# qiyunzhu/woltka

Hardware: AMD Instinct MI355X
Metric: alignment records/sec classified (higher is better)
Workload: dtype u8; 1 GPU; synthetic SAM text of 50M reads x <=16 hits (10.50 GB) resident in HBM, 2M-node taxonomy, ranks phylum,genus,species: device tokenizer per 64 MB block + one weighted histogram per sample (the kernels of `woltka classify`, host link left out); records_per_gpu=250034804, reads_per_gpu=50000000

## Files before the change

woltka_amd/csrc/wk_dtok_fused.hpp:

```cpp
#pragma once
#include "wk_dtok.hpp"
#include "wk_dtok_neighbour.hpp"
#include "wk_dtok_planes.hpp"
#include "wk_dtok_rounds.hpp"

namespace wk {

constexpr uint32_t kFzThreads = 512;
constexpr uint32_t kFzWaves = kFzThreads / kWave;
constexpr uint32_t kFzTile = 16384;
constexpr uint32_t kFzBack = 1024;
constexpr uint32_t kFzFwd = 3072;
constexpr uint32_t kFzWin = kFzTile + kFzBack + kFzFwd;
constexpr uint32_t kFzChunks = kFzWin / 16 + 1;
constexpr uint32_t kFzRounds = kFrMaxRounds;
static_assert(kFrChunks * 16u == kFzWin && kFrTailChunk + 1u == kFzChunks && kFrWaves == kFzWaves && kFrWave == kWave,
              "the dealing covers the window");
constexpr uint32_t kFzLines = 1024;
constexpr uint32_t kFzStreams = 4;
constexpr uint32_t kFzCap = 1024;
static_assert(kFzCap >= kFzLines, "a window's records fit an empty buffer");
static_assert(kFzWin + 32 < 65536, "window offsets fit 16 bits");
constexpr uint32_t kFzCarry = 256;
static_assert(kFzCarry + kFzLines <= kFpMaxLines && kFzThreads % kWave == 0, "a window's owned lines fit the planes, a wave's lines one word");

constexpr uint32_t kDtokSpill = 64;

struct FusedArgs {
    const unsigned char* text;
    uint32_t n;
    uint32_t open_end;
    uint32_t span;
    const struct DictSlot8* dict8;
    const uint4* names16;
    uint32_t dict_mask;
    const unsigned char* arena;
    uint2* unknown;
    uint32_t unknown_cap;
    DtokState* state;
    DtokState* host_state;
    const unsigned long long* backup_prev;
    unsigned long long* backup_next;
    uint32_t* host_seq;
    uint32_t seq;
    StreamSet streams;
    const int32_t* submap;
    uint32_t n_submap;
    uint32_t ablate;
};

static_assert(sizeof(DtokState) % 8 == 0, "the packed totals are aligned");
__device__ __forceinline__ unsigned long long* fz_totals(DtokState* state) { return reinterpret_cast<unsigned long long*>(state + 1); }

__global__ void dtok_fused_begin_kernel(unsigned long long* __restrict__ backup, const unsigned long long* __restrict__ cursor, DtokState* state) {
    if (threadIdx.x < (uint32_t)kMaxStreams) backup[threadIdx.x] = cursor[threadIdx.x];
    if (threadIdx.x == 0) {
        *state = DtokState{0u, 0u, 0ull, 0ull, 0ull, 0u, 0u};
        *fz_totals(state) = 0ull;
    }
}

template <int kCtrl, int kRowMask>
__device__ __forceinline__ uint32_t fz_dpp_add(uint32_t v) {
    return v + (uint32_t)__builtin_amdgcn_update_dpp(0, (int)v, kCtrl, kRowMask, 0xF, false);
}
__device__ __forceinline__ uint32_t fz_wave_scan(uint32_t v) {
    static_assert(kWave == 64, "four rows of sixteen lanes");
    v = fz_dpp_add<0x111, 0xF>(v);
    v = fz_dpp_add<0x112, 0xF>(v);
    v = fz_dpp_add<0x114, 0xF>(v);
    v = fz_dpp_add<0x118, 0xF>(v);
    v = fz_dpp_add<0x142, 0xA>(v);
    v = fz_dpp_add<0x143, 0xC>(v);
    return v;
}
__device__ __forceinline__ uint32_t fz_last_lane(uint32_t v) { return (uint32_t)__builtin_amdgcn_readlane((int)v, kWave - 1); }
__device__ __forceinline__ uint32_t fz_wave_sum(uint32_t v) { return fz_last_lane(fz_wave_scan(v)); }
__device__ __forceinline__ unsigned long long fz_first_lane64(unsigned long long v) {
    return ((unsigned long long)(uint32_t)__builtin_amdgcn_readfirstlane((int)(uint32_t)(v >> 32)) << 32) |
           (uint32_t)__builtin_amdgcn_readfirstlane((int)(uint32_t)v);
}

__device__ __forceinline__ uint4 fz_load_stream(const unsigned char* p) {
    typedef uint32_t u32x4 __attribute__((ext_vector_type(4)));
    const u32x4 v = __builtin_nontemporal_load(reinterpret_cast<const u32x4*>(p));
    return make_uint4(v.x, v.y, v.z, v.w);
}
__device__ __forceinline__ unsigned long long fz_load64(const unsigned char* p) {
    unsigned long long w;
    __builtin_memcpy(&w, p, 8);
    return w;
}
__device__ __forceinline__ uint32_t fz_load32(const unsigned char* p) {
    uint32_t w;
    __builtin_memcpy(&w, p, 4);
    return w;
}
__device__ __forceinline__ unsigned long long fz_eq_bytes(unsigned long long w, unsigned char c) {
    const unsigned long long x = w ^ (0x0101010101010101ull * c);
    return ~(((x & 0x7F7F7F7F7F7F7F7Full) + 0x7F7F7F7F7F7F7F7Full) | x | 0x7F7F7F7F7F7F7F7Full);
}
__device__ __forceinline__ uint32_t fz_marks32(uint32_t w, uint32_t c4) {
    const uint32_t x = w ^ c4;
    return ~(((x & 0x7F7F7F7Fu) + 0x7F7F7F7Fu) | x | 0x7F7F7F7Fu);
}
__device__ __forceinline__ unsigned long long fz_low_bytes(unsigned long long w, uint32_t k) {
    return k >= 8u ? w : (w & ((1ull << (8u * k)) - 1ull));
}

__device__ __forceinline__ unsigned long long fz_hash(const unsigned char* p, uint32_t n) {
    unsigned long long h = 0xcbf29ce484222325ull ^ ((unsigned long long)n * 0x9E3779B97F4A7C15ull);
    while (n >= 8u) {
        h = (h ^ fz_load64(p)) * 0x100000001b3ull;
        h ^= h >> 29;
        p += 8;
        n -= 8u;
    }
    const unsigned long long v = n ? fz_low_bytes(fz_load64(p), n) : 0ull;
    h = (h ^ v) * 0x100000001b3ull;
    h ^= h >> 32;
    h *= 0x9E3779B97F4A7C15ull;
    return h ^ (h >> 29);
}

__device__ __forceinline__ bool fz_same(const unsigned char* x, const unsigned char* y, uint32_t n) {
    while (n >= 8u) {
        if (fz_load64(x) != fz_load64(y)) return false;
        x += 8;
        y += 8;
        n -= 8u;
    }
    return n == 0u || fz_low_bytes(fz_load64(x) ^ fz_load64(y), n) == 0ull;
}

struct FzProbe {
    unsigned long long hv, n0, n1;
    uint32_t h;
    uint2 slot;
};
__device__ __forceinline__ FzProbe fz_probe_begin(const FusedArgs& a, const unsigned char* name, uint32_t rn) {
    FzProbe p;
    p.n0 = p.n1 = 0ull;
    if (rn <= 15u) {
        const unsigned long long lo = fz_low_bytes(fz_load64(name), rn), hi = rn > 8u ? fz_low_bytes(fz_load64(name + 8), rn - 8u) : 0ull;
        p.n0 = lo;
        p.n1 = hi | ((unsigned long long)rn << 56);
        unsigned long long h = 0xcbf29ce484222325ull ^ ((unsigned long long)rn * 0x9E3779B97F4A7C15ull), v = lo;
        if (rn >= 8u) {
            h = (h ^ lo) * 0x100000001b3ull;
            h ^= h >> 29;
            v = hi;
        }
        h = (h ^ v) * 0x100000001b3ull;
        h ^= h >> 32;
        h *= 0x9E3779B97F4A7C15ull;
        p.hv = h ^ (h >> 29);
    } else {
        p.hv = fz_hash(name, rn);
    }
    p.h = (uint32_t)p.hv & a.dict_mask;
    p.slot = reinterpret_cast<const uint2*>(a.dict8)[p.h];
    return p;
}
__device__ __forceinline__ int32_t fz_probe_end(const FusedArgs& a, FzProbe p, const unsigned char* name, uint32_t rn, uint32_t abs_off) {
    for (;;) {
        const int32_t id = (int32_t)p.slot.y;
        if (id < 0) break;
        if (p.slot.x == (uint32_t)(p.hv >> 32)) {
            const uint4 nm = a.names16[id];
            const unsigned long long s0 = ((unsigned long long)nm.y << 32) | nm.x, s1 = ((unsigned long long)nm.w << 32) | nm.z;
            if (rn <= 15u) {
                if (s0 == p.n0 && s1 == p.n1) return id;
            } else if ((nm.w >> 24) == 0xFFu) {
                const unsigned char* full = a.arena + nm.x;
                if (fz_load32(full) == rn && fz_same(name, full + 4, rn)) return id;
            }
        }
        p.h = (p.h + 1u) & a.dict_mask;
        p.slot = reinterpret_cast<const uint2*>(a.dict8)[p.h];
    }
    const uint32_t at = atomicAdd(&a.state->n_unknown, 1u);
    if (at < a.unknown_cap)
        a.unknown[at] = make_uint2(abs_off, rn);
    else
        atomicOr(&a.state->flags, kDtokUnknownFull);
    return kLineUnknown;
}

__device__ bool fz_starts_run_slow(const unsigned char* __restrict__ text, uint32_t at, const unsigned char* q, uint32_t qn) {
    uint32_t pos = at;
    while (pos > 0u) {
        const uint32_t e = pos - 1u;
        uint32_t s = e;
        while (s > 0u && text[s - 1u] != '\n') --s;
        uint32_t tab[3], nt = 0;
        for (uint32_t p = s; p < e && nt < 3u; ++p)
            if (text[p] == '\t') tab[nt++] = p;
        if (nt == 3u && !(tab[2] - tab[1] == 2u && text[tab[1] + 1u] == '*')) {
            if (tab[0] - s != qn) return true;
            for (uint32_t k = 0; k < qn; ++k)
                if (text[s + k] != q[k]) return true;
            return false;
        }
        pos = s;
    }
    return true;
}

constexpr uint32_t kFiSubj = (1u << 23) - 1u;
constexpr uint32_t kFiMateShift = 24;
constexpr uint32_t kFiMapped = 1u << 26;
constexpr uint32_t kFiStart = 1u << 27;
constexpr uint32_t kFiUndecided = 1u << 28;
constexpr uint32_t kFiExcl = 1u << 29;
constexpr uint32_t kFiDropped = 1u << 30;
constexpr uint32_t kFiRead = kFiMapped | (3u << kFiMateShift);
constexpr uint32_t kFiKey = kFiRead | kFiSubj;
constexpr uint32_t kFzPad = 8;
static_assert(kFwWave == kWave && kFwWaves == kFzWaves, "the line pass's dealing is this workgroup's");

__device__ __forceinline__ uint32_t fz_octet(uint32_t z_lo, uint32_t z_hi) { return (((z_lo >> 7) | (z_hi >> 3)) * 0x00204081u >> 21) & 255u; }

__device__ __forceinline__ uint32_t fz_newlines16(uint4 v) {
    return fz_octet(fz_marks32(v.x, 0x0A0A0A0Au), fz_marks32(v.y, 0x0A0A0A0Au)) | (fz_octet(fz_marks32(v.z, 0x0A0A0A0Au), fz_marks32(v.w, 0x0A0A0A0Au)) << 8);
}

__device__ __forceinline__ uint32_t fz_tabs32(const unsigned char* p, unsigned long long* q0 = nullptr, unsigned long long* q1 = nullptr) {
    unsigned long long w[4];
#pragma unroll
    for (uint32_t i = 0; i < 4; ++i) w[i] = fz_load64(p + 8u * i);
    uint32_t m = 0;
#pragma unroll
    for (uint32_t i = 0; i < 4; ++i)
        m |= fz_octet(fz_marks32((uint32_t)w[i], 0x09090909u), fz_marks32((uint32_t)(w[i] >> 32), 0x09090909u)) << (8u * i);
    if (q0) {
        *q0 = w[0];
        *q1 = w[1];
    }
    return m;
}

template <bool kMeasure>
__device__ __forceinline__ void dtok_fused_body(const FusedArgs& a) {
    __shared__ __attribute__((aligned(16))) unsigned char txt[kFzChunks * 16 + 32];
    __shared__ uint16_t ls[kFzLines + 2];
    __shared__ uint16_t f_qn[kFzLines];
    __shared__ __attribute__((aligned(16))) uint32_t info_[kFzPad + kFzCarry + kFzLines + kFzPad + 8];
    __shared__ uint32_t carry[kFzCarry];
    __shared__ unsigned long long planes[kFpPlanes][kFpWords];
    __shared__ uint32_t rbuf[kFzStreams][kFzCap];
    __shared__ unsigned long long fill_packed;
    static_assert(kFzStreams <= 4 && kFzCap + kFzThreads < 65536, "four 16-bit counts");
    __shared__ unsigned long long gbase[kFzStreams];
    __shared__ uint32_t wtot[kFzWaves];
    __shared__ unsigned long long gbase_out[kMaxStreams];
    __shared__ unsigned long long wg_totals;
    __shared__ uint32_t own[5];
    __shared__ uint32_t wg_flags;
    uint32_t* const info = info_ + kFzPad + kFzCarry;

    const uint32_t tid = threadIdx.x, lane = tid & (kWave - 1), wave = tid / kWave;
    const uint32_t wave_s = (uint32_t)__builtin_amdgcn_readfirstlane((int)wave);
    const uint32_t n_streams = a.streams.n_streams;
    const uint32_t ablate = kMeasure ? a.ablate : 0u;
    const int32_t* const submap = a.submap;
    unsigned long long fill = 0ull;
    if (tid == 0) fill_packed = 0ull;
    if (tid < 4u) reinterpret_cast<uint32_t*>(txt + kFrTailChunk * 16u)[tid] = 0u;
    if (tid == 0) wg_flags = 0u;
// ... 130 lines not shown
            }
        }
        __syncthreads();
        const uint32_t trail = too_many ? wpos : w0 + (uint32_t)__builtin_amdgcn_readfirstlane((int)(uint32_t)ls[total_nl]);
        if (!too_many && last_win && trail >= t0 && trail < t1) my_flags |= kDtokSpill;
        const uint32_t first_line = mode != 0u || w0 == 0u ? 0u : 1u;
        const uint32_t n_lines = too_many ? 0u : total_nl;
        if (tid == 0 && first_line) info[0] = 0u;

        const bool first_starts = nc == 0u && (mode == 1u || wpos == 0u);
        for (uint32_t k0 = first_line; k0 < n_lines; k0 += kFwTrip) {
            const uint32_t k = fw_line(k0, wave, lane);
            const bool has = fw_has(k, first_line, n_lines), owner = !fw_witness(lane);
            uint32_t word = 0, s = 0, qn = 0, rb = 0, rn = 0;
            unsigned long long q0 = 0ull, q1 = 0ull;
            if (has) {
                s = ls[k];
                const uint32_t e = (uint32_t)ls[k + 1] - 1u;
                uint32_t tab[3] = {0, 0, 0}, nt = 0;
                if (!(ablate & 256u)) {
                    uint32_t m = fz_tabs32(txt + s, &q0, &q1);
                    if (e - s < 32u) m &= (1u << (e - s)) - 1u;
                    nt = min((uint32_t)__popc(m), 3u);
                    tab[0] = s + (uint32_t)__ffs((int)m) - 1u;
                    m &= m - 1u;
                    tab[1] = s + (uint32_t)__ffs((int)m) - 1u;
                    m &= m - 1u;
                    tab[2] = s + (uint32_t)__ffs((int)m) - 1u;
                    for (uint32_t p = s + 32u; nt < 3u && p < e; p += 32u) {
                        m = fz_tabs32(txt + p);
                        if (e - p < 32u) m &= (1u << (e - p)) - 1u;
                        for (; m && nt < 3u; m &= m - 1u) {
                            const uint32_t q = p + (uint32_t)__ffs((int)m) - 1u;
                            if (nt == 0u)
                                tab[0] = q;
                            else if (nt == 1u)
                                tab[1] = q;
                            else
                                tab[2] = q;
                            ++nt;
                        }
                    }
                }
                if (ablate & 16u) {
                } else if (nt < 3u) {
                    my_flags |= kDtokShortLine;
                } else {
                    const uint32_t fl = tab[1] - tab[0] - 1u;
                    const unsigned long long fw = fz_load64(txt + tab[0] + 1u);
                    uint32_t flag = 0;
                    bool digits = fl >= 1u && fl <= 6u;
                    for (uint32_t i = 0; i < fl && i < 6u; ++i) {
                        const uint32_t d = ((uint32_t)(fw >> (8u * i)) & 0xFFu) - (uint32_t)'0';
                        digits &= d <= 9u;
                        flag = flag * 10u + d;
                    }
                    rb = tab[1] + 1u;
                    rn = tab[2] - rb;
                    if (!digits) {
                        my_flags |= kDtokShortLine;
                    } else if (rn == 1u && txt[rb] == '*') {
                    } else {
                        const uint32_t mate = (flag >> 6) & 3u;
                        if (mate == 3u) my_flags |= kDtokBothMates;
                        word = kFiMapped | (mate << kFiMateShift);
                        qn = tab[0] - s;
                        if (owner) f_qn[k] = (uint16_t)qn;
                    }
                }
            }
            const bool mapped = (word & kFiMapped) != 0u, look = owner && mapped && w0 + s >= t0;
            const unsigned char* const name = txt + rb;
            FzProbe probe;
            if (look && !(ablate & 1u)) probe = fz_probe_begin(a, name, rn);
            const FnLine me = has ? fn_line(mapped, qn, q0, q1) : fn_no_line();
            FnLine prev;
            prev.meta = (uint32_t)__builtin_amdgcn_update_dpp(0, (int)me.meta, 0x138 , 0xF, 0xF, false);
#pragma unroll
            for (uint32_t i = 0; i < 4; ++i) prev.b[i] = (uint32_t)__builtin_amdgcn_update_dpp(0, (int)me.b[i], 0x138, 0xF, 0xF, false);
            const uint32_t verdict = ((ablate & 8u) || (first_starts && k == first_line)) ? (uint32_t)kFnStarts : (uint32_t)fn_verdict(prev, me);
            const bool start = look && verdict == kFnStarts;
            const unsigned long long b_und = __ballot(look && verdict == kFnUndecided);
            if (lane == 0 && b_und != 0ull) own[4] = 1u;
            if (look) {
                int32_t sid = (ablate & 1u) ? (int32_t)(fz_load32(name + 4) % 1000u) : fz_probe_end(a, probe, name, rn, w0 + rb);
                bool excluded = false;
                if (submap && sid >= 0) {
                    if ((uint32_t)sid < a.n_submap) {
                        sid = submap[sid];
                        if (sid == kLineExcluded) {
                            excluded = true;
                            sid = 0;
                        }
                    } else {
                        my_flags |= kDtokSpill;
                        sid = -1;
                    }
                }
                word |= (start ? kFiStart : 0u) | (verdict == kFnUndecided ? kFiUndecided : 0u) | (excluded ? kFiExcl : 0u) |
                        (sid < 0 ? kFiSubj : ((uint32_t)sid & kFiSubj));
            }
            if (has && owner) info[k] = word;
            const unsigned long long b_all = __ballot(start), b_in = __ballot(start && w0 + s < t1), b_out = b_all & ~b_in;
            if (lane == 0 && b_all) {
                if (b_in) atomicMin(&own[0], k + (uint32_t)__builtin_ctzll(b_in));
                if (b_out) atomicMin(&own[1], k + (uint32_t)__builtin_ctzll(b_out));
                atomicMax(&own[2], k + 63u - (uint32_t)__builtin_clzll(b_all));
            }
        }
        __syncthreads();
        if (__builtin_amdgcn_readfirstlane((int)own[4])) {
        for (uint32_t k0 = first_line; k0 < n_lines; k0 += kFzThreads) {
            const uint32_t k = k0 + tid;
            const uint32_t mk = k < n_lines ? info[k] : 0u;
            const bool und = (mk & kFiUndecided) != 0u;
            bool start = false;
            if (__ballot(und) != 0ull) {
                if (und) {
                    uint32_t j = k;
                    bool found = false;
                    while (j > first_line) {
                        --j;
                        if (info[j] & kFiMapped) {
                            found = true;
                            break;
                        }
                    }
                    if (found)
                        start = f_qn[j] != f_qn[k] || !fz_same(txt + ls[k], txt + ls[j], f_qn[k]);
                    else if (nc)
                        start = f_qn[k] != cq_len || !fz_same(txt + ls[k], a.text + cq_pos, cq_len);
                    else if (mode == 1u || wpos == 0u)
                        start = true;
                    else
                        start = fz_starts_run_slow(a.text, w0 + ls[first_line], txt + ls[k], f_qn[k]);
                }
            }
            if (mk & kFiUndecided) {
                info[k] = (mk & ~kFiUndecided) | (start ? kFiStart : 0u);
                if (start) {
                    atomicMin(&own[w0 + ls[k] < t1 ? 0 : 1], k);
                    atomicMax(&own[2], k);
                }
            }
        }
        __syncthreads();
        }
        const uint32_t o0 = (uint32_t)__builtin_amdgcn_readfirstlane((int)own[0]), o1 = (uint32_t)__builtin_amdgcn_readfirstlane((int)own[1]);
        const uint32_t last = (uint32_t)__builtin_amdgcn_readfirstlane((int)own[2]);
        const uint32_t lpos = w0 + (uint32_t)__builtin_amdgcn_readfirstlane((int)(uint32_t)ls[o0 != 0xFFFFFFFFu ? last : 0u]);
        const bool has_first = nc != 0u || o0 != 0xFFFFFFFFu;
        const int32_t first_own = nc ? -(int32_t)nc : (int32_t)o0;
        int32_t ka = 0, kb = 0;
        uint32_t next = 0u, next_mode = 0u, nc_next = 0u;
        bool more = false, again = false, put_aside = false;
        if (too_many) {
            if ((ablate & (32u | 512u)) && !last_win) {
                next = w1;
                next_mode = 2u;
                more = true;
            }
        } else if (o1 != 0xFFFFFFFFu) {
            kb = (int32_t)o1;
            ka = has_first ? first_own : kb;
        } else if (to_end) {
            kb = (int32_t)n_lines;
            ka = has_first ? first_own : kb;
        } else if (last_win && a.span <= kFzTile) {
// ... 197 lines not shown
```

woltka_amd/csrc/woltka_hip.hip:

```cpp
#include <hip/hip_runtime.h>

#include <algorithm>
#include <atomic>
#include <ctime>
#include <chrono>
#include <cstdarg>
#include <cstdio>
#include <cstdlib>
#include <cstring>
#include <map>
#include <new>
#include <mutex>
#include <string>
#include <vector>

#include "../../include/woltka_hip.h"
#include "../../include/woltka_hip_measure.h"
#include "wk_classify.hpp"
#include "wk_cover.hpp"
#include "wk_device.hpp"
#include "wk_dtok.hpp"
#include "wk_demux.hpp"
#include "wk_strata_reads.hpp"
#include "wk_dtok_fused.hpp"
// ... 200 lines not shown
    int tally_per_cu = 3;
    int tally_slots = 1024;
    int use_tally = 1;
    int match_lds = 1;
    bool listed_only = false;
    int bins_ring = 4;
    DevBuf w_slab, w_hi, w_invalid;
    DevBuf w_wide, w_wide_plan;
    int weigh_wide = 0;
    int weigh_wide_wgs = 0;
    size_t w_hi_clean = 0;
    DevBuf sz_rows, sz_counts, sz_scal;
    DevBuf lr_table;
    int64_t sz_n = 0, sz_flushes = 0;
    DevBuf c_rk[2], rk_left[2], rk_totals;
    bool rk_valid[2] = {false, false};
    int64_t rk_reads[2] = {0, 0}, rk_records[2] = {0, 0};
    int64_t stage_serial = 0, rows_serial = 0, rk1_stage = -1, rk1_rows = -1;
    int64_t stat_extra_reads = 0, stat_extra_records = 0;
    bool rows_any_invalid = false;
    DevBuf c_words;
    DevBuf w_stream[kMaxStreams], w_cursor, w_stage, w_backup, w_backup2;
    void* w_backup_cur = nullptr;
    bool fz_chain = false;
    int fz_parity = 0;
    DevBuf w_backup3;
    struct LagSlot {
        int buf = -1;
        const char* src = nullptr;
        uint32_t n = 0;
        bool open_end = false;
        int ring = 0;
        uint32_t lines_est = 0;
        int host_slot = 0;
        hipEvent_t ev = nullptr;
        uint32_t seq = 0;
    };
    LagSlot lag[2];
    int lag_count = 0;
    hipEvent_t lag_ev[2] = {nullptr, nullptr};
    int lag_next_ev = 0;
    int fz_back_streak = 0, fz_skip = 0;
    bool count_ahead = true;
    bool lag_poll = true;
    uint32_t lag_seq = 0;
    bool lag_enabled = true;
    int w_streams = 0;
    bool w_sliced = false;
    bool w_counts_known = false;
    unsigned long long w_count[kMaxStreams] = {};
    int64_t w_records = 0, w_reads = 0;
    std::vector<wk_job> w_jobs;
    int32_t w_group = 0;
    bool w_open = false;
    struct HostReg {
        const char* p;
        size_t n;
    };
    std::mutex reg_mu;
    std::vector<HostReg> regs;
    int w_mode = 0;
    bool w_mixed_entry = false;
    int rank_serial = 0;
    int free_per_cu = 2, free_threads = 1024, free_slots = 4096;
    int32_t max_gene_feature = 0;
    int use_range_log = 1;
    int words_keep = 0;
    static constexpr int kStageSlots = 8;
    hipEvent_t slot_ev[kStageSlots] = {};
    bool slot_busy[kStageSlots] = {};
    std::vector<void*> host_blocks;
    std::mutex host_mu;
    static constexpr int kTextBufs = 192;
    static constexpr int kSlabBufs = 16;
    static constexpr size_t kTextStride = ((size_t)66 << 20) + 256;
    DevBuf d_textslab[kTextBufs / kSlabBufs];
    enum : unsigned char { kBufFree = 0, kBufCopied = 1, kBufScanning = 2, kBufPending = 3 };
    TextBuf text_buf[kTextBufs];
    std::mutex copy_mu;
    std::mutex slab_mu;
    unsigned long long copy_seq_next = 1;
    unsigned long long* copy_newlines = nullptr;
    uint32_t* di_any_host = nullptr;
    DevBuf d_tiles, d_tile_off, d_lines, d_lsubj, d_lmeta, d_start, d_first, d_unknown, d_state, d_dict, d_dict2, d_names16, d_arena, d_submap;
    bool dt_mapped = false;
    bool dt_submap_on = false;
    bool dt_has_excl = false;
    uint32_t dt_submap_n = 0;
    DevBuf d_lbeg, d_lend, d_llen, d_lscan, d_gmap;
    bool dt_extra = false;
    DevBuf cv_key[2], cv_end[2], cv_reach, cv_hist, cv_tiles, cv_tile_off, cv_state, cv_stage[3];
    bool cv_open = false;
    int cv_cur = 0;
    int64_t cv_cap = 0;
    int64_t cv_cap_opt = 0;
    int64_t cv_tail = 0;
    int64_t cv_merged = 0;
    int64_t cv_ub = 0;
    bool cv_stale = false;
    CoverState cv_seen{};
    uint32_t cv_line_next = 0;
    struct ResidentText {
        const char* host;
        uint32_t n;
        unsigned char* dev;
        unsigned long long* tile_off;
        unsigned long long n_newlines;
    };
    std::vector<ResidentText> resident;
    DevBuf di_blob, di_meta, di_out, di_status;
    const unsigned char* dt_text = nullptr;
    int dt_fmt = 0;
    uint32_t dt_n = 0, dt_lines = 0, dt_dict_mask = 0;
    int32_t dt_dict_names = -1;
    const wk_tok* dt_dict_tok = nullptr;
    bool dt_ready = false;
    hipStream_t copy_stream = nullptr, count_stream = nullptr;
    bool dt_detached = false;
    int64_t dt_expect_bytes = 0, w_expect = 0;
    unsigned char* host_back = nullptr;
    static constexpr int kBackSlots = 4, kBackBytes = 256;
    struct MapTables {
        DevBuf slot_of_subject, slot_order, shown_off, shown;
        int32_t n_subjects = 0, n_slots = 0;
    };
    MapTables rm[WK_MAX_JOBS];
    DevBuf rm_line, rm_len, rm_text;
    DevBuf s_text, s_lines, s_tab, s_vlen, s_hash, s_label, s_slots, s_labels, s_label_text, s_label_group, s_state, s_tiles, s_tile_off;
    uint32_t s_n = 0, s_n_lines = 0, s_mask = 0;
    bool s_ready = false;
    bool s_use = false;
    DevBuf dx_tab, dx_name_off, dx_arena, dx_group, dx_met, dx_pend, dx_pend_list, dx_state, dx_lsamp, dx_out;
    std::vector<DemuxSlot> dx_tab_host;
    std::vector<uint2> dx_name_off_host;
    std::vector<unsigned char> dx_arena_host;
    std::vector<int64_t> dx_pend_off;
    std::vector<int32_t> dx_pend_len;
    std::vector<char> dx_pend_blob;
    bool dx_on = false;
    bool dx_looked = false;
    bool dx_runs = false;
    int dx_status = 1;
    bool dx_chunk = false;
    bool dx_hits = false;
    DevBuf dx_rsamp;
    int32_t dx_groups_n = 0;
    uint64_t dx_hash_mask = 0;
    int64_t dx_max_opt = 0;
    bool dt_keep_reads = false;
    bool dt_emitted = false;
    uint32_t dt_emit_reads = 0;
    int64_t rm_bytes = 0;
    int range_parts_opt = 0;
    int use_streams = 1;
    int use_subject_bins = 1;
    int use_hot_bins = 1;
};

namespace {

int fail(wk_ctx* ctx, int code, const char* fmt, ...) {
    char buf[512];
    va_list ap;
    va_start(ap, fmt);
    vsnprintf(buf, sizeof buf, fmt, ap);
    va_end(ap);
    if (ctx)
// ... 554 lines not shown
                                 hipFuncAttributeMaxDynamicSharedMemorySize, 144 * 1024)) != hipSuccess ||
        (e = hipFuncSetAttribute(reinterpret_cast<const void*>(&classify_single_kernel<true, false, 2, false, true>),
                                 hipFuncAttributeMaxDynamicSharedMemorySize, 144 * 1024)) != hipSuccess ||
        (e = hipFuncSetAttribute(reinterpret_cast<const void*>(&classify_single_kernel<false, true, kPerReadItems, true>),
                                 hipFuncAttributeMaxDynamicSharedMemorySize, 144 * 1024)) != hipSuccess ||
        (e = hipFuncSetAttribute(reinterpret_cast<const void*>(&classify_single_kernel<false, false, kPerReadItems, true>),
                                 hipFuncAttributeMaxDynamicSharedMemorySize, 144 * 1024)) != hipSuccess ||
        (e = hipFuncSetAttribute(reinterpret_cast<const void*>(&weigh_bins_kernel<4>),
                                 hipFuncAttributeMaxDynamicSharedMemorySize, (int)kBinsMaxLds)) != hipSuccess ||
        (e = hipFuncSetAttribute(reinterpret_cast<const void*>(&weigh_bins_kernel<4, true>),
                                 hipFuncAttributeMaxDynamicSharedMemorySize, (int)kBinsMaxLds)) != hipSuccess ||
        (e = hipFuncSetAttribute(reinterpret_cast<const void*>(&weigh_bins_kernel<6, true>),
                                 hipFuncAttributeMaxDynamicSharedMemorySize, (int)kBinsMaxLds)) != hipSuccess ||
        (e = hipFuncSetAttribute(reinterpret_cast<const void*>(&weigh_bins_kernel<8, true>),
                                 hipFuncAttributeMaxDynamicSharedMemorySize, (int)kBinsMaxLds)) != hipSuccess ||
        (e = hipFuncSetAttribute(reinterpret_cast<const void*>(&weigh_bins_kernel<3>),
                                 hipFuncAttributeMaxDynamicSharedMemorySize, (int)kBinsMaxLds)) != hipSuccess ||
        (e = hipFuncSetAttribute(reinterpret_cast<const void*>(&weigh_bins_kernel<6>),
                                 hipFuncAttributeMaxDynamicSharedMemorySize, (int)kBinsMaxLds)) != hipSuccess ||
        (e = hipFuncSetAttribute(reinterpret_cast<const void*>(&weigh_bins_kernel<8>),
                                 hipFuncAttributeMaxDynamicSharedMemorySize, (int)kBinsMaxLds)) != hipSuccess ||
        (e = hipFuncSetAttribute(reinterpret_cast<const void*>(&weigh_streams_kernel<4>),
                                 hipFuncAttributeMaxDynamicSharedMemorySize, (int)kBinsMaxLds)) != hipSuccess ||
        (e = hipFuncSetAttribute(reinterpret_cast<const void*>(&weigh_streams_kernel<6>),
                                 hipFuncAttributeMaxDynamicSharedMemorySize, (int)kBinsMaxLds)) != hipSuccess ||
        (e = hipFuncSetAttribute(reinterpret_cast<const void*>(&weigh_streams_kernel<8>),
                                 hipFuncAttributeMaxDynamicSharedMemorySize, (int)kBinsMaxLds)) != hipSuccess ||
        (e = hipFuncSetAttribute(reinterpret_cast<const void*>(&weigh_wide_kernel<4>),
                                 hipFuncAttributeMaxDynamicSharedMemorySize, (int)kBinsMaxLds)) != hipSuccess ||
        (e = hipFuncSetAttribute(reinterpret_cast<const void*>(&sized_bins_kernel<4>),
                                 hipFuncAttributeMaxDynamicSharedMemorySize, (int)kBinsMaxLds)) != hipSuccess ||
        (e = hipFuncSetAttribute(reinterpret_cast<const void*>(&weigh_merge_kernel),
                                 hipFuncAttributeMaxDynamicSharedMemorySize, 144 * 1024)) != hipSuccess ||
        (e = hipFuncSetAttribute(reinterpret_cast<const void*>(&classify_tiled_kernel),
                                 hipFuncAttributeMaxDynamicSharedMemorySize, 144 * 1024)) != hipSuccess ||
        (e = hipFuncSetAttribute(reinterpret_cast<const void*>(&match_hits_kernel<true, true>),
                                 hipFuncAttributeMaxDynamicSharedMemorySize, 156 * 1024)) != hipSuccess ||
        (e = hipFuncSetAttribute(reinterpret_cast<const void*>(&match_hits_kernel<true, false>),
                                 hipFuncAttributeMaxDynamicSharedMemorySize, 156 * 1024)) != hipSuccess ||
        (e = hipFuncSetAttribute(reinterpret_cast<const void*>(&range_merge_kernel),
                                 hipFuncAttributeMaxDynamicSharedMemorySize, 144 * 1024)) != hipSuccess ||
        (e = hipFuncSetAttribute(reinterpret_cast<const void*>(&partition_merge_kernel),
                                 hipFuncAttributeMaxDynamicSharedMemorySize, 144 * 1024)) != hipSuccess) {
        int rc = fail(nullptr, WK_E_HIP, "hipFuncSetAttribute(max dynamic LDS) failed: %s", hipGetErrorString(e));
        wk_destroy(c);
        return rc;
    }
    if (const char* nf = getenv("WOLTKA_NO_FUSED")) c->use_fused = (nf[0] && nf[0] != '0') ? 0 : 1;
    if (const char* nl = getenv("WOLTKA_NO_LAG")) c->lag_enabled = !(nl[0] && nl[0] != '0');
    if (const char* lp = getenv("WOLTKA_LAG_POLL")) c->lag_poll = lp[0] && lp[0] != '0';
    if (const char* sm = getenv("WOLTKA_STRIPES_MIN"))
        if (sm[0]) c->stripes_min_hits = std::max<long long>(0, atoll(sm));
    *out = c;
    return WK_OK;
}

void wk_destroy(wk_ctx* c) {
    if (!c) return;
    DeviceGuard guard(c->device);
    if (c->stream) (void)hipStreamSynchronize(c->stream);
    DevBuf* bufs[] = {&c->nodes, &c->rank_code, &c->gene4, &c->g_grid, &c->g_first, &c->g_goff, &c->g_shift,
                      &c->tkeys, &c->tvals, &c->c_subj, &c->c_qoff, &c->c_group, &c->o_genome, &c->o_beg,
                      &c->o_end, &c->o_len, &c->o_hoff, &c->o_cnt, &c->o_ub, &c->o_first2, &c->o_poff, &c->o_pairs, &c->o_qoff,
                      &c->o_tile_sum, &c->o_tile_off, &c->scalars, &c->stat_block, &c->log, &c->subj_feat, &c->subj_rows, &c->dense_slab, &c->plog, &c->plog_cnt, &c->left_mask, &c->left_list, &c->first_slab, &c->w_slab, &c->w_hi, &c->w_invalid, &c->sz_rows, &c->sz_counts, &c->sz_scal, &c->lr_table, &c->c_rk[0], &c->c_rk[1], &c->rk_left[0], &c->rk_left[1], &c->rk_totals, &c->f_rank, &c->f_sparse, &c->f_dense, &c->w_renum, &c->f_log, &c->f_log_cnt, &c->f_partial, &c->f_part_used, &c->w_tmp, &c->assign_out, &c->fetch_k, &c->fetch_v};
    for (DevBuf* b : bufs) b->release();
    for (wk_ctx::StreamTables& T : c->st)
        for (DevBuf* b : {&T.dsparse, &T.dparent, &T.dself, &T.rnode, &T.subj_node, &T.subj_rank}) b->release();
    c->c_words.release();
    for (DevBuf* b : {&c->di_blob, &c->di_meta, &c->di_out, &c->di_status}) b->release();
    for (DevBuf& b : c->w_stream) b.release();
    c->w_wide.release();
    c->w_wide_plan.release();
    c->w_backup2.release();
    c->w_backup3.release();
    for (hipEvent_t& e : c->lag_ev)
        if (e) (void)hipEventDestroy(e);
    for (TextBuf& b : c->text_buf) {
        for (DevBuf* d : {&b.tiles, &b.tile_off, &b.di_comp, &b.di_meta, &b.di_status, &b.own}) d->release();
        for (hipEvent_t ev : {b.ev, b.ev0, b.evm})
            if (ev) (void)hipEventDestroy(ev);
    }
    for (DevBuf& slab : c->d_textslab) slab.release();
    for (DevBuf* b : {&c->d_tiles, &c->d_tile_off, &c->d_lines, &c->d_lsubj, &c->d_lmeta, &c->d_start, &c->d_first, &c->d_unknown, &c->d_lbeg, &c->d_lend, &c->d_llen, &c->d_lscan, &c->d_gmap,
                      &c->d_state, &c->d_dict, &c->d_dict2, &c->d_names16, &c->d_arena, &c->d_submap, &c->cv_key[0], &c->cv_key[1], &c->cv_end[0], &c->cv_end[1],
                      &c->cv_reach, &c->cv_hist, &c->cv_tiles, &c->cv_tile_off, &c->cv_state, &c->cv_stage[0], &c->cv_stage[1], &c->cv_stage[2],
                      &c->dx_tab, &c->dx_name_off, &c->dx_arena, &c->dx_group, &c->dx_met, &c->dx_pend, &c->dx_pend_list, &c->dx_state, &c->dx_lsamp, &c->dx_out, &c->dx_rsamp})
        b->release();
    for (wk_ctx::ResidentText& r : c->resident) {
        (void)hipFree(r.dev);
        (void)hipFree(r.tile_off);
    }
    c->resident.clear();
    for (void* hp : c->host_blocks) (void)hipHostFree(hp);
    if (c->host_back) (void)hipHostFree(c->host_back);
    for (const wk_ctx::HostReg& r : c->regs) (void)hipHostUnregister(const_cast<char*>(r.p));
    c->regs.clear();
    if (c->di_any_host) (void)hipHostFree(c->di_any_host);
    if (c->copy_stream) (void)hipStreamDestroy(c->copy_stream);
    if (c->count_stream) (void)hipStreamDestroy(c->count_stream);
    if (c->res_ev) (void)hipEventDestroy(c->res_ev);
    for (hipEvent_t ev : c->slot_ev)
        if (ev) (void)hipEventDestroy(ev);
    for (DevBuf& b : c->rank_tab) b.release();
    for (auto& kv : c->ktimers)
        if (kv.second.b) (void)hipEventDestroy(kv.second.b);
    if (c->kt_step) (void)hipEventDestroy(c->kt_step);
    if (c->t0) (void)hipEventDestroy(c->t0);
    if (c->t1) (void)hipEventDestroy(c->t1);
    if (c->stream) (void)hipStreamDestroy(c->stream);
    delete c;
}

int wk_device_name(const wk_ctx* c, char* buf, size_t cap) {
    if (!c || !buf || cap == 0) return WK_E_ARG;
    snprintf(buf, cap, "%s (%s, %d CUs)", c->prop.name, c->prop.gcnArchName, c->prop.multiProcessorCount);
    return WK_OK;
}

int wk_sync(wk_ctx* c) {
    if (!c) return WK_E_ARG;
    DeviceGuard guard(c->device);
    HIP_TRY(c, hipStreamSynchronize(c->stream));
    if (c->count_stream) HIP_TRY(c, hipStreamSynchronize(c->count_stream));
    return WK_OK;
}

int wk_set_option(wk_ctx* c, const char* name, int64_t value) {
    if (!c || !name) return WK_E_ARG;
    if (!strcmp(name, "gene_index_pairs")) {
        c->gene_index_opt = value != 0;
        return WK_OK;
    }
    if (!strcmp(name, "dtok_count_ahead")) {
        c->count_ahead = value != 0;
        return WK_OK;
    }
    if (!strcmp(name, "cover_cap_rows")) {
        if (value != 0 && (value < kCoverCapMin || value > kCoverCapMax))
            return fail(c, WK_E_ARG, "cover_cap_rows must be 0 or in [%lld, %lld]", (long long)kCoverCapMin, (long long)kCoverCapMax);
        c->cv_cap_opt = value;
        return WK_OK;
    }
    if (!strcmp(name, "demux_hash_mask")) {
        c->dx_hash_mask = (uint64_t)value;
        return WK_OK;
    }
    if (!strcmp(name, "demux_max_samples")) {
        if (value < 0 || value > (int64_t)kDemuxMaxSamples) return fail(c, WK_E_ARG, "demux_max_samples must be in [0, %u]", kDemuxMaxSamples);
        c->dx_max_opt = value;
        return WK_OK;
    }
    return fail(c, WK_E_ARG, "unknown option '%s' (launch shapes and ablation switches: wk_tune)", name);
}

int wk_tune(wk_ctx* c, const char* name, int64_t value) {
    if (!c || !name) return WK_E_ARG;
    if (!strcmp(name, "lds_slots")) {
        if (value < 64 || value > 8192 || (value & (value - 1))) return fail(c, WK_E_ARG, "lds_slots must be a power of two in [64, 8192]");
        c->lds_slots = (int)value;
        return WK_OK;
    }
    if (!strcmp(name, "blocks_per_cu")) {
        if (value < 1 || value > 32) return fail(c, WK_E_ARG, "blocks_per_cu must be in [1, 32]");
        c->blocks_per_cu = (int)value;
        return WK_OK;
    }
    if (!strcmp(name, "threads")) {
// ... 1700 lines not shown
    } else if (n_records > 0) {
        HIP_TRY(c, hipMemcpyAsync(c->c_words.as<uint32_t>() + c->w_records, words, (size_t)n_records * 4, hipMemcpyHostToDevice, c->stream));
    }
    if (slot >= 0) {
        if (!c->slot_ev[slot]) HIP_TRY(c, hipEventCreateWithFlags(&c->slot_ev[slot], hipEventDisableTiming));
        HIP_TRY(c, hipEventRecord(c->slot_ev[slot], c->stream));
        c->slot_busy[slot] = true;
    }
    if (n_records > 0 && c->w_mode == 0) {
        hipLaunchKernelGGL(words_partition_kernel, dim3((unsigned)((n_records + 256 * kScatterItems - 1) / (256 * kScatterItems))), dim3(256), 0, c->stream,
                           c->w_stage.as<uint32_t>(), (uint32_t)n_records, stream_set(c));
        HIP_TRY(c, hipGetLastError());
        c->w_counts_known = false;
    }
    {
        const int rct = words_translate(c, c->w_records, n_records);
        if (rct) return rct;
    }
    if (slot < 0) HIP_TRY(c, hipStreamSynchronize(c->stream));
    c->w_records += n_records;
    c->w_reads += n_reads;
    return WK_OK;
}

int wk_words_wait(wk_ctx* c, int slot) {
    if (!c || slot < 0 || slot >= wk_ctx::kStageSlots) return WK_E_ARG;
    if (!c->slot_busy[slot]) return WK_OK;
    DeviceGuard guard(c->device);
    HIP_TRY(c, hipEventSynchronize(c->slot_ev[slot]));
    c->slot_busy[slot] = false;
    return WK_OK;
}

int wk_words_pending(wk_ctx* c, int64_t* n_records, int64_t* n_reads) {
    if (!c) return WK_E_ARG;
    if (n_records) *n_records = c->w_open ? c->w_records : 0;
    if (n_reads) *n_reads = c->w_open ? c->w_reads : 0;
    return WK_OK;
}


static int dtok_mirror_dict(wk_ctx* c, const wk_tok* tok) {
    const int32_t n = wkx_tok_n_names(tok);
    if (c->dt_dict_tok == tok && c->dt_dict_names == n) return WK_OK;
    uint32_t slots = 1024;
    while (slots < 2u * (uint32_t)n + 2u) slots <<= 1;
    std::vector<DictSlot> tab(slots, DictSlot{0ull, -1, 0u});
    std::string arena;
    arena.reserve((size_t)n * 16 + 16);
    for (int32_t id = 0; id < n; ++id) {
        const char* p;
        uint32_t len;
        uint64_t hv;
        wkx_tok_name(tok, id, &p, &len, &hv);
        const uint32_t off = (uint32_t)arena.size();
        arena.append(reinterpret_cast<const char*>(&len), 4);
        arena.append(p, len);
        uint32_t h = (uint32_t)hv & (slots - 1);
        while (tab[h].id >= 0) h = (h + 1) & (slots - 1);
        tab[h] = DictSlot{(unsigned long long)hv, id, off};
    }
    arena.append(16, '\0');
    int rc;
    if ((rc = upload(c, c->d_dict, tab.data(), tab.size() * sizeof(DictSlot)))) return rc;
    if ((rc = upload(c, c->d_arena, arena.data(), arena.size()))) return rc;
    std::vector<DictSlot8> tab8(slots, DictSlot8{0u, -1});
    std::vector<unsigned char> names16((size_t)std::max(n, 1) * 16, 0);
    for (uint32_t h = 0; h < slots; ++h) {
        if (tab[h].id < 0) continue;
        tab8[h] = DictSlot8{(uint32_t)(tab[h].hash >> 32), tab[h].id};
        uint32_t len;
        std::memcpy(&len, arena.data() + tab[h].off, 4);
        unsigned char* rec = names16.data() + (size_t)tab[h].id * 16;
        if (len <= 15) {
            std::memcpy(rec, arena.data() + tab[h].off + 4, len);
            rec[15] = (unsigned char)len;
        } else {
            std::memcpy(rec, &tab[h].off, 4);
            rec[15] = 0xFF;
        }
    }
    if ((rc = upload(c, c->d_dict2, tab8.data(), tab8.size() * sizeof(DictSlot8)))) return rc;
    if ((rc = upload(c, c->d_names16, names16.data(), names16.size()))) return rc;
    HIP_TRY(c, hipStreamSynchronize(c->stream));
    c->dt_dict_mask = slots - 1;
    c->dt_dict_names = n;
    c->dt_dict_tok = tok;
    return WK_OK;
}

static DtokArgs dtok_args(wk_ctx* c) {
    DtokArgs a{};
    a.text = c->dt_text;
    a.n = c->dt_n;
    a.fmt = (uint32_t)c->dt_fmt;
    a.line_start = c->d_lines.as<uint32_t>();
    a.n_lines = c->dt_lines;
    a.lsubj = c->d_lsubj.as<int32_t>();
    a.lmeta = c->d_lmeta.as<uint32_t>();
    a.dict = c->d_dict.as<DictSlot>();
    a.dict_mask = c->dt_dict_mask;
    a.arena = c->d_arena.as<unsigned char>();
    a.dict8 = c->d_dict2.as<DictSlot8>();
    a.names16 = c->d_names16.as<uint4>();
    a.unknown = c->d_unknown.as<uint2>();
    a.unknown_cap = (uint32_t)(c->d_unknown.cap / 8);
    a.is_start = c->d_start.as<unsigned char>();
    a.is_first = c->d_first.as<unsigned char>();
    a.state = c->d_state.as<DtokState>();
    a.lbeg = c->d_lbeg.as<int32_t>();
    a.lend = c->d_lend.as<int32_t>();
    a.llen = c->d_llen.as<uint32_t>();
    a.line_scan = c->d_lscan.as<unsigned long long>();
    a.submap = c->dt_submap_on ? c->d_submap.as<int32_t>() : nullptr;
    a.n_submap = c->dt_submap_n;
    return a;
}

static void count_newlines(const unsigned char* text, uint32_t n, unsigned long long* tiles, unsigned long long* tile_off,
                           unsigned long long* total, hipStream_t stream) {
    const uint32_t n_tiles = (n + kDtokTile - 1) / kDtokTile;
    hipLaunchKernelGGL(dtok_count_kernel, dim3(n_tiles), dim3(kDtokThreads), 0, stream, text, n, tiles);
    hipLaunchKernelGGL(tile_scan_kernel, dim3(1), dim3(1024), 0, stream, tiles, tile_off, (int64_t)n_tiles, total);
}

static hipError_t copy_text_async(wk_ctx* c, void* dst, const char* src, size_t n, hipStream_t stream) {
    std::vector<size_t> cuts{0, n};
    {
        std::lock_guard<std::mutex> lock(c->reg_mu);
        for (const wk_ctx::HostReg& r : c->regs) {
            if (r.p > src && r.p < src + n) cuts.push_back((size_t)(r.p - src));
            if (r.p + r.n > src && r.p + r.n < src + n) cuts.push_back((size_t)(r.p + r.n - src));
        }
    }
    std::sort(cuts.begin(), cuts.end());
    for (size_t i = 0; i + 1 < cuts.size(); ++i) {
        if (cuts[i + 1] == cuts[i]) continue;
        const hipError_t e = hipMemcpyAsync((char*)dst + cuts[i], src + cuts[i], cuts[i + 1] - cuts[i], hipMemcpyHostToDevice, stream);
        if (e != hipSuccess) return e;
    }
    return hipSuccess;
}

int wk_host_register(wk_ctx* c, const void* p, size_t bytes) {
    if (!c || !p || !bytes) return WK_E_ARG;
    DeviceGuard guard(c->device);
    const hipError_t e = hipHostRegister(const_cast<void*>(p), bytes, hipHostRegisterReadOnly);
    if (e != hipSuccess) {
        (void)hipGetLastError();
        return fail(c, WK_E_HIP, "hipHostRegister(%zu bytes) failed: %s", bytes, hipGetErrorString(e));
    }
    std::lock_guard<std::mutex> lock(c->reg_mu);
    c->regs.push_back(wk_ctx::HostReg{(const char*)p, bytes});
    return WK_OK;
}

int wk_host_unregister(wk_ctx* c, const void* p) {
    if (!c || !p) return WK_E_ARG;
    {
        std::lock_guard<std::mutex> lock(c->reg_mu);
        auto it = std::find_if(c->regs.begin(), c->regs.end(), [&](const wk_ctx::HostReg& r) { return r.p == (const char*)p; });
        if (it == c->regs.end()) return fail(c, WK_E_ARG, "not a registered range");
        c->regs.erase(it);
    }
    DeviceGuard guard(c->device);
    HIP_TRY(c, hipHostUnregister(const_cast<void*>(p)));
// ... 323 lines not shown

int wk_dtok_fused_counts(wk_ctx* c, int64_t* done, int64_t* handed_back) {
    if (!c || !done || !handed_back) return WK_E_ARG;
    *done = c->fused_blocks;
    *handed_back = c->fused_fallbacks;
    return WK_OK;
}

int wk_text_clear(wk_ctx* c) {
    if (!c) return WK_E_ARG;
    DeviceGuard guard(c->device);
    for (wk_ctx::ResidentText& r : c->resident) {
        (void)hipFree(r.dev);
        (void)hipFree(r.tile_off);
    }
    c->resident.clear();
    return WK_OK;
}

int wk_dtok_subject_map(wk_ctx* c, const int32_t* map, int32_t n) {
    if (!c || n < 0 || (n > 0 && !map)) return WK_E_ARG;
    DeviceGuard guard(c->device);
    c->dt_submap_on = map != nullptr;
    if (map && n == 0) HIP_TRY(c, c->d_submap.reserve(64));
    bool excl = false;
    if (n > 0) {
        for (int32_t i = 0; i < n; ++i) {
            if (map[i] == kLineExcluded)
                excl = true;
            else if (map[i] < 0)
                return fail(c, WK_E_ARG, "a subject map holds subject indices (or -4: excluded)");
        }
        HIP_TRY(c, hipStreamSynchronize(c->stream));
        const int rc = upload(c, c->d_submap, map, (size_t)n * 4);
        if (rc) return rc;
        HIP_TRY(c, hipStreamSynchronize(c->stream));
    }
    c->dt_submap_n = (uint32_t)n;
    c->dt_has_excl = excl;
    return WK_OK;
}

int wk_dtok_format(wk_ctx* c, int fmt) {
    if (!c) return WK_E_ARG;
    if (fmt != WK_FMT_SAM && fmt != WK_FMT_MAP && fmt != WK_FMT_B6O && fmt != WK_FMT_PAF)
        return fail(c, WK_E_ARG, "the device tokenizer takes SAM, simple maps, BLAST tabular text and PAF");
    c->dt_fmt = fmt;
    return WK_OK;
}

static DevBuf& fz_bk(wk_ctx* c, int i) { return i == 0 ? c->w_backup : i == 1 ? c->w_backup2 : c->w_backup3; }

static unsigned fused_spans(const wk_ctx* c, uint32_t n, uint32_t* span) {
    const uint64_t wgs = (uint64_t)c->prop.multiProcessorCount * (uint64_t)c->fused_per_cu;
    const uint64_t share = (((uint64_t)n + wgs - 1) / wgs + 15u) & ~(uint64_t)15u;
    *span = (uint32_t)std::max<uint64_t>(share, 4096u);
    return (unsigned)(((uint64_t)n + *span - 1) / *span);
}

static int dtok_emit_launch(wk_ctx* c, bool* ordered_out, unsigned long long* totals);
static int dtok_emit_finish(wk_ctx* c, bool keep, bool ordered, DtokState st, unsigned long long totals, int64_t* n_reads,
                            int64_t* n_records);

static const wk_ctx::ResidentText* resident_text(const wk_ctx* c, const char* src, uint32_t n) {
    const wk_ctx::ResidentText* res = nullptr;
    for (const wk_ctx::ResidentText& r : c->resident)
        if (r.host == src && r.n == n) res = &r;
    return res;
}

static hipError_t dtok_scratch_reserve(wk_ctx* c) {
    const hipError_t e = c->d_state.reserve(sizeof(DtokState) + 64);
    return e != hipSuccess ? e : c->d_unknown.reserve((size_t)(1 << 20) * 8);
}

static void words_expect_from_block(wk_ctx* c) {
    if (c->dt_expect_bytes <= 0 || c->w_expect != 0 || c->dt_n == 0) return;
    const double lines = (double)c->dt_expect_bytes * ((double)c->dt_lines / (double)c->dt_n) * 1.08 + (double)c->dt_lines;
    c->w_expect = (int64_t)std::min(lines, (double)(1ll << 30));
}

static bool fused_eligible(const wk_ctx* c, const wk_tok* tok) {
    return c->use_fused && c->dt_fmt == WK_FMT_SAM && c->w_open && c->w_mode == 0 && !c->dt_keep_reads &&
           wkx_tok_n_names(tok) < (1 << 23) - 1;
}

static int fused_launch(wk_ctx* c, const StreamSet& streams, const unsigned char* text, uint32_t n, bool open_end, int ring, int host_slot,
                        uint32_t seq) {
    static_assert(sizeof(DtokState) <= 128 && wk_ctx::kBackBytes >= 132, "the slot's second half holds the block's sequence number");
    FusedArgs fa{};
    const unsigned grid = fused_spans(c, n, &fa.span);
    if (fa.span % 16u) return fail(c, WK_E_ARG, "spans of the one-kernel tokenizer are multiples of 16 bytes");
    HIP_TRY(c, dtok_scratch_reserve(c));
    for (int i = 0; i < 3; ++i) HIP_TRY(c, fz_bk(c, i).reserve(kMaxStreams * 8));
    fa.text = text;
    fa.n = n;
    fa.open_end = open_end ? 1u : 0u;
    fa.dict8 = c->d_dict2.as<DictSlot8>();
    fa.names16 = c->d_names16.as<uint4>();
    fa.dict_mask = c->dt_dict_mask;
    fa.arena = c->d_arena.as<unsigned char>();
    fa.unknown = c->d_unknown.as<uint2>();
    fa.unknown_cap = (uint32_t)(c->d_unknown.cap / 8);
    fa.state = c->d_state.as<DtokState>();
    unsigned char* slot = c->host_back + (size_t)host_slot * wk_ctx::kBackBytes;
    fa.host_state = reinterpret_cast<DtokState*>(slot);
    fa.backup_prev = fz_bk(c, ring).as<unsigned long long>();
    fa.backup_next = fz_bk(c, (ring + 1) % 3).as<unsigned long long>();
    fa.host_seq = seq ? reinterpret_cast<uint32_t*>(slot + 128) : nullptr;
    fa.seq = seq;
    fa.streams = streams;
    fa.submap = c->dt_submap_on ? c->d_submap.as<int32_t>() : nullptr;
    fa.n_submap = c->dt_submap_n;
    fa.ablate = c->fused_ablate;
    c->w_counts_known = false;
    KernelTimer* kf = ktimer_begin(c, "dtok_fused");
    if (!c->fz_chain)
        hipLaunchKernelGGL(dtok_fused_begin_kernel, dim3(1), dim3(64), 0, c->stream, fz_bk(c, ring).as<unsigned long long>(),
                           (const unsigned long long*)streams.cursor, fa.state);
    if (c->fused_ablate != 0u)
        hipLaunchKernelGGL(dtok_fused_measure_kernel, dim3(grid), dim3(kFzThreads), 0, c->stream, fa);
    else
        hipLaunchKernelGGL(dtok_fused_kernel, dim3(grid), dim3(kFzThreads), 0, c->stream, fa);
    ktimer_end(c, kf);
    HIP_TRY(c, hipGetLastError());
    return WK_OK;
}

static uint32_t fz_kept(wk_ctx* c, const DtokState& st, uint32_t n, bool open_end) {
    const uint32_t lines = (uint32_t)st.n_lines + (open_end ? 1u : 0u);
    c->dt_lines = lines;
    c->dt_lpb = (double)lines / (double)n;
    c->fused_streak = true;
    c->fz_back_streak = 0;
    ++c->fused_blocks;
    return lines;
}

static void fz_handed_back(wk_ctx* c) {
    c->fused_streak = false;
    c->fz_chain = false;
    ++c->fused_fallbacks;
    c->fz_back_streak = std::min(c->fz_back_streak + 1, 6);
    if (c->fz_back_streak >= 2) c->fz_skip = 1 << (c->fz_back_streak - 1);
}

struct ScanBlock {
    wk_tok* tok;
    const char* src;
    uint32_t n;
    bool extra;
    int64_t* n_lines;
    int* status;
    int* emit;
    int64_t* emitted;
    enum { kResident, kCopiedAhead, kCopiedNow } where;
    const wk_ctx::ResidentText* res;
    int k;
    bool counted;
    bool open_end;
    bool fuse;
    bool have_count;
    unsigned long long n_newlines;
    const unsigned long long* tile_off;
    uint32_t lines;
    KernelTimer* kt;
    std::chrono::steady_clock::time_point lap_t;
};

static void scan_lap(wk_ctx* c, ScanBlock& s, int i) {
    const auto now = std::chrono::steady_clock::now();
    c->lap_x[i] += std::chrono::duration<double>(now - s.lap_t).count();
    s.lap_t = now;
}

static void scan_reply_emitted(wk_ctx* c, const ScanBlock& s, int64_t n_reads, int64_t n_records) {
    *s.status = 0;
    *s.n_lines = s.lines;
    *s.emit = 1;
    s.emitted[0] = n_reads;
    s.emitted[1] = n_records;
    c->dt_ready = false;
}
// ... 2156 lines not shown
```

Before: 17.58 billion records/s.

## Replace linear-probe dictionary with 4-way tagged buckets and wave-uniform probe loop

The fused tokenizer's name dictionary changes from a linear-probing table of 8-byte slots to a bucketed table of 16-byte buckets. Each bucket holds four 32-bit entries that pack a 9-bit hash tag with a 23-bit id. One vector load now checks four candidates, and the probe loop is restructured so the wave advances together under ballots, tracking refuted candidates per lane. The aim is fewer dependent global loads and less divergence per lookup. In exchange the host builds and uploads a second table, and the short tag may send more false-positive name comparisons to the names16 table.

```diff
diff --git a/woltka_amd/csrc/wk_dtok_dict.hpp b/woltka_amd/csrc/wk_dtok_dict.hpp
--- /dev/null
+++ b/woltka_amd/csrc/wk_dtok_dict.hpp
@@ -0,0 +1,45 @@
+#pragma once
+#include <cstdint>
+
+#if defined(__HIPCC__) || defined(__CUDACC__)
+#define WK_FD_FN __host__ __device__ __forceinline__
+#else
+#define WK_FD_FN inline
+#endif
+
+namespace wk {
+
+constexpr uint32_t kFdIdBits = 23, kFdIdMask = (1u << kFdIdBits) - 1u;
+constexpr uint32_t kFdMaxId = kFdIdMask - 1u;
+constexpr uint32_t kFdEmpty = 0xFFFFFFFFu;
+constexpr uint32_t kFdWays = 4;
+
+WK_FD_FN uint32_t fd_buckets(uint32_t slots) { return slots / 2u; }
+WK_FD_FN uint32_t fd_tagword(unsigned long long hv) { return (uint32_t)(hv >> 55) << kFdIdBits; }
+WK_FD_FN uint32_t fd_home(unsigned long long hv, uint32_t bucket_mask) { return (uint32_t)hv & bucket_mask; }
+WK_FD_FN uint32_t fd_next(uint32_t bucket, uint32_t bucket_mask) { return (bucket + 1u) & bucket_mask; }
+WK_FD_FN uint32_t fd_entry(uint32_t tagword, uint32_t id) { return tagword | id; }
+WK_FD_FN uint32_t fd_id(uint32_t entry) { return entry & kFdIdMask; }
+WK_FD_FN bool fd_tagged(uint32_t entry, uint32_t tagword) { return (entry ^ tagword) < kFdIdMask; }
+WK_FD_FN uint32_t fd_match(uint32_t e0, uint32_t e1, uint32_t e2, uint32_t e3, uint32_t tagword) {
+    return (fd_tagged(e0, tagword) ? 1u : 0u) | (fd_tagged(e1, tagword) ? 2u : 0u) | (fd_tagged(e2, tagword) ? 4u : 0u) |
+           (fd_tagged(e3, tagword) ? 8u : 0u);
+}
+WK_FD_FN uint32_t fd_pick(uint32_t e0, uint32_t e1, uint32_t e2, uint32_t e3, uint32_t m) {
+    return (m & 1u) ? e0 : (m & 2u) ? e1 : (m & 4u) ? e2 : e3;
+}
+WK_FD_FN bool fd_full(uint32_t e3) { return e3 != kFdEmpty; }
+
+WK_FD_FN uint32_t fd_insert(uint32_t* table, uint32_t bucket_mask, unsigned long long hv, uint32_t id) {
+    uint32_t b = fd_home(hv, bucket_mask), trips = 1u;
+    while (fd_full(table[kFdWays * b + kFdWays - 1u])) {
+        b = fd_next(b, bucket_mask);
+        ++trips;
+    }
+    uint32_t* e = table + kFdWays * b;
+    while (*e != kFdEmpty) ++e;
+    *e = fd_entry(fd_tagword(hv), id);
+    return trips;
+}
+
+}
diff --git a/woltka_amd/csrc/wk_dtok_fused.hpp b/woltka_amd/csrc/wk_dtok_fused.hpp
--- a/woltka_amd/csrc/wk_dtok_fused.hpp
+++ b/woltka_amd/csrc/wk_dtok_fused.hpp
@@ -1,5 +1,6 @@
 #pragma once
 #include "wk_dtok.hpp"
+#include "wk_dtok_dict.hpp"
 #include "wk_dtok_neighbour.hpp"
 #include "wk_dtok_planes.hpp"
 #include "wk_dtok_rounds.hpp"
@@ -31,9 +32,9 @@
     uint32_t n;
     uint32_t open_end;
     uint32_t span;
-    const struct DictSlot8* dict8;
+    const uint4* dictb;
     const uint4* names16;
-    uint32_t dict_mask;
+    uint32_t bucket_mask;
     const unsigned char* arena;
     uint2* unknown;
     uint32_t unknown_cap;
@@ -134,12 +135,13 @@
 }
 
 struct FzProbe {
-    unsigned long long hv, n0, n1;
-    uint32_t h;
-    uint2 slot;
+    unsigned long long n0, n1;
+    uint32_t tagword, b;
+    uint4 bucket;
 };
 __device__ __forceinline__ FzProbe fz_probe_begin(const FusedArgs& a, const unsigned char* name, uint32_t rn) {
     FzProbe p;
+    unsigned long long hv;
     p.n0 = p.n1 = 0ull;
     if (rn <= 15u) {
         const unsigned long long lo = fz_low_bytes(fz_load64(name), rn), hi = rn > 8u ? fz_low_bytes(fz_load64(name + 8), rn - 8u) : 0ull;
@@ -154,37 +156,63 @@
         h = (h ^ v) * 0x100000001b3ull;
         h ^= h >> 32;
         h *= 0x9E3779B97F4A7C15ull;
-        p.hv = h ^ (h >> 29);
+        hv = h ^ (h >> 29);
     } else {
-        p.hv = fz_hash(name, rn);
-    }
-    p.h = (uint32_t)p.hv & a.dict_mask;
-    p.slot = reinterpret_cast<const uint2*>(a.dict8)[p.h];
+        hv = fz_hash(name, rn);
+    }
+    p.tagword = fd_tagword(hv);
+    p.b = fd_home(hv, a.bucket_mask);
+    p.bucket = a.dictb[p.b];
     return p;
 }
-__device__ __forceinline__ int32_t fz_probe_end(const FusedArgs& a, FzProbe p, const unsigned char* name, uint32_t rn, uint32_t abs_off) {
-    for (;;) {
-        const int32_t id = (int32_t)p.slot.y;
-        if (id < 0) break;
-        if (p.slot.x == (uint32_t)(p.hv >> 32)) {
+__device__ __forceinline__ int32_t fz_probe_end(const FusedArgs& a, FzProbe p, bool look, const unsigned char* name, uint32_t rn,
+                                                uint32_t abs_off) {
+    int32_t sid = kLineUnknown;
+    bool pend = look;
+    uint32_t refuted = 0u;
+    while (__ballot(pend) != 0ull) {
+        uint32_t m = 0u;
+        for (;;) {
+            bool on = false;
+            if (pend) {
+                m = fd_match(p.bucket.x, p.bucket.y, p.bucket.z, p.bucket.w, p.tagword) & ~refuted;
+                on = m == 0u && fd_full(p.bucket.w);
+                pend = m != 0u || on;
+            }
+            if (__ballot(on) == 0ull) break;
+            if (on) {
+                p.b = fd_next(p.b, a.bucket_mask);
+                p.bucket = a.dictb[p.b];
+                refuted = 0u;
+            }
+        }
+        if (pend) {
+            const int32_t id = (int32_t)fd_id(fd_pick(p.bucket.x, p.bucket.y, p.bucket.z, p.bucket.w, m));
             const uint4 nm = a.names16[id];
             const unsigned long long s0 = ((unsigned long long)nm.y << 32) | nm.x, s1 = ((unsigned long long)nm.w << 32) | nm.z;
+            bool same = false;
             if (rn <= 15u) {
-                if (s0 == p.n0 && s1 == p.n1) return id;
+                same = s0 == p.n0 && s1 == p.n1;
             } else if ((nm.w >> 24) == 0xFFu) {
                 const unsigned char* full = a.arena + nm.x;
-                if (fz_load32(full) == rn && fz_same(name, full + 4, rn)) return id;
-            }
-        }
-        p.h = (p.h + 1u) & a.dict_mask;
-        p.slot = reinterpret_cast<const uint2*>(a.dict8)[p.h];
-    }
-    const uint32_t at = atomicAdd(&a.state->n_unknown, 1u);
-    if (at < a.unknown_cap)
-        a.unknown[at] = make_uint2(abs_off, rn);
-    else
-        atomicOr(&a.state->flags, kDtokUnknownFull);
-    return kLineUnknown;
+                same = fz_load32(full) == rn && fz_same(name, full + 4, rn);
+            }
+            if (same) {
+                sid = id;
+                pend = false;
+            } else {
+                refuted |= m & (0u - m);
+            }
+        }
+    }
+    if (look && sid < 0) {
+        const uint32_t at = atomicAdd(&a.state->n_unknown, 1u);
+        if (at < a.unknown_cap)
+            a.unknown[at] = make_uint2(abs_off, rn);
+        else
+            atomicOr(&a.state->flags, kDtokUnknownFull);
+    }
+    return sid;
 }
 
 __device__ bool fz_starts_run_slow(const unsigned char* __restrict__ text, uint32_t at, const unsigned char* q, uint32_t qn) {
@@ -481,8 +509,9 @@
             const bool start = look && verdict == kFnStarts;
             const unsigned long long b_und = __ballot(look && verdict == kFnUndecided);
             if (lane == 0 && b_und != 0ull) own[4] = 1u;
+            const int32_t found = (ablate & 1u) ? (int32_t)(fz_load32(name + 4) % 1000u) : fz_probe_end(a, probe, look, name, rn, w0 + rb);
             if (look) {
-                int32_t sid = (ablate & 1u) ? (int32_t)(fz_load32(name + 4) % 1000u) : fz_probe_end(a, probe, name, rn, w0 + rb);
+                int32_t sid = found;
                 bool excluded = false;
                 if (submap && sid >= 0) {
                     if ((uint32_t)sid < a.n_submap) {
diff --git a/woltka_amd/csrc/woltka_hip.hip b/woltka_amd/csrc/woltka_hip.hip
--- a/woltka_amd/csrc/woltka_hip.hip
+++ b/woltka_amd/csrc/woltka_hip.hip
@@ -306,7 +306,7 @@
     unsigned long long copy_seq_next = 1;
     unsigned long long* copy_newlines = nullptr;
     uint32_t* di_any_host = nullptr;
-    DevBuf d_tiles, d_tile_off, d_lines, d_lsubj, d_lmeta, d_start, d_first, d_unknown, d_state, d_dict, d_dict2, d_names16, d_arena, d_submap;
+    DevBuf d_tiles, d_tile_off, d_lines, d_lsubj, d_lmeta, d_start, d_first, d_unknown, d_state, d_dict, d_dict2, d_dictb, d_names16, d_arena, d_submap;
     bool dt_mapped = false;
     bool dt_submap_on = false;
     bool dt_has_excl = false;
@@ -1027,7 +1027,7 @@
     }
     for (DevBuf& slab : c->d_textslab) slab.release();
     for (DevBuf* b : {&c->d_tiles, &c->d_tile_off, &c->d_lines, &c->d_lsubj, &c->d_lmeta, &c->d_start, &c->d_first, &c->d_unknown, &c->d_lbeg, &c->d_lend, &c->d_llen, &c->d_lscan, &c->d_gmap,
-                      &c->d_state, &c->d_dict, &c->d_dict2, &c->d_names16, &c->d_arena, &c->d_submap, &c->cv_key[0], &c->cv_key[1], &c->cv_end[0], &c->cv_end[1],
+                      &c->d_state, &c->d_dict, &c->d_dict2, &c->d_dictb, &c->d_names16, &c->d_arena, &c->d_submap, &c->cv_key[0], &c->cv_key[1], &c->cv_end[0], &c->cv_end[1],
                       &c->cv_reach, &c->cv_hist, &c->cv_tiles, &c->cv_tile_off, &c->cv_state, &c->cv_stage[0], &c->cv_stage[1], &c->cv_stage[2],
                       &c->dx_tab, &c->dx_name_off, &c->dx_arena, &c->dx_group, &c->dx_met, &c->dx_pend, &c->dx_pend_list, &c->dx_state, &c->dx_lsamp, &c->dx_out, &c->dx_rsamp})
         b->release();
@@ -2894,6 +2894,19 @@
     }
     if ((rc = upload(c, c->d_dict2, tab8.data(), tab8.size() * sizeof(DictSlot8)))) return rc;
     if ((rc = upload(c, c->d_names16, names16.data(), names16.size()))) return rc;
+    std::vector<uint32_t> tabb;
+    if (n <= 0 || (uint32_t)(n - 1) <= kFdMaxId) {
+        const uint32_t buckets = fd_buckets(slots);
+        tabb.assign((size_t)kFdWays * buckets, kFdEmpty);
+        for (int32_t id = 0; id < n; ++id) {
+            const char* p;
+            uint32_t len;
+            uint64_t hv;
+            wkx_tok_name(tok, id, &p, &len, &hv);
+            fd_insert(tabb.data(), buckets - 1u, (unsigned long long)hv, (uint32_t)id);
+        }
+        if ((rc = upload(c, c->d_dictb, tabb.data(), tabb.size() * sizeof(uint32_t)))) return rc;
+    }
     HIP_TRY(c, hipStreamSynchronize(c->stream));
     c->dt_dict_mask = slots - 1;
     c->dt_dict_names = n;
@@ -3383,7 +3396,7 @@
 
 static bool fused_eligible(const wk_ctx* c, const wk_tok* tok) {
     return c->use_fused && c->dt_fmt == WK_FMT_SAM && c->w_open && c->w_mode == 0 && !c->dt_keep_reads &&
-           wkx_tok_n_names(tok) < (1 << 23) - 1;
+           (uint32_t)wkx_tok_n_names(tok) <= kFdMaxId;
 }
 
 static int fused_launch(wk_ctx* c, const StreamSet& streams, const unsigned char* text, uint32_t n, bool open_end, int ring, int host_slot,
@@ -3397,9 +3410,9 @@
     fa.text = text;
     fa.n = n;
     fa.open_end = open_end ? 1u : 0u;
-    fa.dict8 = c->d_dict2.as<DictSlot8>();
+    fa.dictb = c->d_dictb.as<uint4>();
     fa.names16 = c->d_names16.as<uint4>();
-    fa.dict_mask = c->dt_dict_mask;
+    fa.bucket_mask = fd_buckets(c->dt_dict_mask + 1u) - 1u;
     fa.arena = c->d_arena.as<unsigned char>();
     fa.unknown = c->d_unknown.as<uint2>();
     fa.unknown_cap = (uint32_t)(c->d_unknown.cap / 8);
```

Result: faster. 17.76 billion records/s (median of 6 runs) (+1.0%).
